# zahraamselim/compressed-rag-suite

Measured on AMD Instinct MI355X. Metric: queries/sec over N-vector corpus (exact cosine top-k; Recall@10 vs the exact fp32 ranking), higher is better.
Workload: dtype f16 x f16 -> f32; 1 GPU; c4; corpus_rows=10000000, rows_per_gpu=10000000, dim=384, queries_per_batch=64, distinct_queries_in_flight=2048, lanes=1 encoder + 1 search (encoder kernels <= 48 KB of LDS); 4 batches per sweep, batches_per_encoder_forward=16, searches_per_graph=4, top_k=10, k_scan=24, slab=f16, refine_fp32=True, exact_escalation=True, encoder_in_step=True, engine=rag._engine.RetrievalEngine (the object ContextRetriever.retrieve_batch drives), encoder=all-MiniLM-L6-v2 shape, seeded random weights

## Files before the change

### compressed-rag-suite_amd/csrc/scan.h

```cpp
#pragma once
#include <hip/hip_runtime.h>
#include <stdint.h>

namespace crs {

struct ScanArgs {
  const _Float16* q;
  const void* slab;
  const float* scales;
  float* part_scores;
  int* part_rows;
  unsigned* tau_shared;
  unsigned long long* stamps;
  int n_rows;
  int n_tiles;
  int nq;
  int k;
  int sched;
  int boot;
  int kp;
  int nwg;
  int nqb;
  unsigned* ticket;
  int t_dyn;
  int dyn_mask;
  int nt;
};

struct ExactWs {
  float* thr;
  int* cnt;
  int* done;
  int64_t* lists;
};

int refine_launch(const _Float16* q16, int nq, int pdim, const _Float16* slab, int n_rows, const float* win_s,
                  const int64_t* win, int k, int tile_rows, int64_t id_base, float* out_s, int64_t* out_i, hipStream_t stream);

int refine_i8_launch(const _Float16* q16, int nq, int pdim, const void* slab, const float* scales, int n_rows, const float* win_s,
                     const int64_t* win, int k, int tile_rows, int64_t id_base, float* out_s, int64_t* out_i, hipStream_t stream);

int scan_tile_rows(int pdim);
int scan_i8_tile_rows();
int scan_wg_per_cu();
bool scan_share_tau();
int scan_launch_f16(const ScanArgs& a, int pdim, int nwg, hipStream_t stream);
int scan_launch_i8(const ScanArgs& a, int pdim, int slots, hipStream_t stream);
int scan_tb_wg_per_cu(int pdim, int nw);
bool scan_tb_has_8_waves(int pdim);
int scan_launch_tb(const ScanArgs& a, int pdim, int nw, int slots, hipStream_t stream);
int scan_ticket_zero(unsigned* ticket, hipStream_t stream);
int scan_tb_long_chain_slots(int pdim, int nw, int k);
int scan_i8_long_chain_slots(int pdim, int k);
int scan_wide_waves(int nq, int k, int pdim);
bool scan_wide_streamed(int k);
int scan_wide_wg_per_cu(int nw, int pdim);
int scan_wide_slots(int k);
int scan_wide_tile_rows(int nw, int pdim);
int scan_launch_wide(const ScanArgs& a, int pdim, int nw, hipStream_t stream);

int scan_w1_queries_per_wg(int nq, int k, int pdim);
int scan_launch_w1(const ScanArgs& a, int pdim, hipStream_t stream);

int merge_slices(int nlists, int k_in);
int merge_launch_i32(const float* scores, const int* rows, int nlists, int nq, int k_in, int k_out,
                     int64_t id_base, float* out_scores, int64_t* out_ids, float* inter_s, int64_t* inter_i, hipStream_t stream);
int merge_launch_i64(const float* scores, const int64_t* ids, int nlists, int nq, int k_in, int k_out,
                     float* out_scores, int64_t* out_ids, hipStream_t stream);

int merge_launch_wire(const void* wire, size_t block_bytes, size_t scores_off, int nlists, int nq, int k_in, int k_out,
                      float* out_scores, int64_t* out_ids, hipStream_t stream);

int merge_sorted_launch_i64(const float* scores, const int64_t* ids, int nlists, int nq, int k_in, int k_out, float* out_scores,
                            int64_t* out_ids, hipStream_t stream);
int merge_sorted_launch_wire(const void* wire, size_t block_bytes, size_t scores_off, int nlists, int nq, int k_in, int k_out,
                             float* out_scores, int64_t* out_ids, hipStream_t stream);

int mmr_order_launch(const float* vecs, int64_t n_rows, int dim, const int64_t* rows, const double* rel, const int* counts, int nq,
                     int m_max, double lam, int* order, hipStream_t stream);

int rerank_lexical_launch(const float* scores, const int64_t* rows, int nq, int m_max, const int64_t* doc_off, const int* doc_tok,
                          int64_t n_rows, int64_t n_doc_tok, const int64_t* q_off, const int* q_tok, int64_t n_q_tok, const int* q_norm,
                          int k, double threshold, int* order, int* out_count, double* sim, double* rr, int* reranked, hipStream_t stream);

int token_match_launch(const float* a, const int* len_a, int seq_a, const float* b, const int* len_b, int seq_b, int n_pairs, int hidden,
                       const float* w_a, const float* w_b, float* out, hipStream_t stream);

int refine_f32_launch(const float* q32, int nq, int dim, const float* shadow, int64_t n_rows, int64_t id_base,
                      const int64_t* cand, int k_in, int k_out, float* out_s, int64_t* out_i, hipStream_t stream);
int slab_append_launch(const float* emb, int64_t n, int dim, int pdim, int slab_type, void* slab,
                       float* scales, float* shadow, int64_t row0, float* row_err_max, hipStream_t stream);
int queries_to_f16_launch(const float* q, int nq, int dim, int pdim, _Float16* out, hipStream_t stream);
int score_rows_launch(const float* q32, int nq, int dim, const float* shadow, int64_t n_rows, int64_t id_base, int k, const int64_t* ids,
                      float* scores, hipStream_t stream);
int rescore_launch(const float* q32, int nq, int dim, const float* shadow, int64_t n_rows,
                   int64_t id_base, int k, float* scores, int64_t* ids, hipStream_t stream);

bool finish_fits(int nlists, int kp, int kc, int tile_rows, int pdim);
int finish_cert_launch(const float* part_s, const int* part_r, int nlists, int kp, const _Float16* q16, int nq, int pdim,
                       const _Float16* slab, int n_rows, int tile_rows, const float* q32, int dim, const float* shadow, int64_t id_base,
                       int kc, int k_out, float err_rows, float* cand_s, int64_t* cand_i, float* out_s, int64_t* out_i, int* status,
                       const ExactWs& ws, hipStream_t stream);

float exact_err_arith(int dim, int pdim);
float exact_err_rows_bound(int dim, int slab_type);
int refine_cert_launch(const float* q32, const _Float16* q16, int nq, int dim, int pdim, int slab_type, const float* shadow,
                       int64_t n_rows, int64_t id_base, const int64_t* cand, const float* cand_s, int k_in, int k_out,
                       float err_rows, float* out_s, int64_t* out_i, int* status, const ExactWs& ws, hipStream_t stream);
int escalate_launch(const float* q32, const _Float16* q16, int nq, int dim, int pdim, int slab_type, const void* slab,
                    const float* scales, const float* shadow, int64_t n_rows, int64_t id_base, int k_out, float* out_s,
                    int64_t* out_i, int* status, const ExactWs& ws, int cap, int cus, hipStream_t stream);

int large_k_max_parts();
int large_cert_launch(const float* q32, const _Float16* q16, int nq, int dim, int pdim, int slab_type, const float* shadow, int64_t n_rows,
                      int64_t id_base, const int64_t* cand, const float* cand_s, int parts, int64_t chunk_rows, int k_out, float err_rows,
                      float* out_s, int64_t* out_i, int* status, const ExactWs& ws, hipStream_t stream);

}
```

### compressed-rag-suite_amd/csrc/scan_common.h

```cpp
#pragma once
#include <hip/hip_runtime.h>
#include <stdint.h>

#include "scan.h"
#include "lds_dma.h"

#define CRS_NSTREAMS (a.nwg)
#define CRS_QBLOCK (crs::grid_qblock(a))
#define CRS_STREAM (crs::grid_stream(a))

namespace crs {
namespace {

typedef _Float16 f16x8 __attribute__((ext_vector_type(8)));
typedef float f32x4 __attribute__((ext_vector_type(4)));
typedef unsigned u32x4 __attribute__((ext_vector_type(4)));

__device__ __forceinline__ int grid_qblock(const ScanArgs& a) {
  const int b = (int)blockIdx.x;
  if (a.nqb == 1) return 0;
  if (a.nwg & 7) return b % a.nqb;
  return (b >> 3) % a.nqb;
}
__device__ __forceinline__ int grid_stream(const ScanArgs& a) {
  const int b = (int)blockIdx.x;
  if (a.nqb == 1) return b;
  if (a.nwg & 7) return b / a.nqb;
  return ((b >> 3) / a.nqb) * 8 + (b & 7);
}


#ifdef CRS_STAMPS
#define CRS_STAMP(slot)                                                                          \
  do {                                                                                           \
    if (a.stamps && (threadIdx.x & 63) == 0) {                                                   \
      const unsigned long long t_ = __builtin_amdgcn_s_memtime();                               \
      a.stamps[((size_t)CRS_STREAM * 4 + (threadIdx.x >> 6)) * 64 + (slot)] = t_;                \
    }                                                                                            \
  } while (0)
#define CRS_STAMP_REAL(slot)                                                                     \
  do {                                                                                           \
    if (a.stamps && (threadIdx.x & 63) == 0)                                                     \
      a.stamps[((size_t)CRS_STREAM * 4 + (threadIdx.x >> 6)) * 64 + (slot)] = __builtin_amdgcn_s_memrealtime(); \
  } while (0)
#else
#define CRS_STAMP(slot) do {} while (0)
#define CRS_STAMP_REAL(slot) do {} while (0)

#endif

#ifdef CRS_STAMPS
#define WP_DECL unsigned long long wp_[12] = {0, 0, 0, 0, 0, 0, 0, 0, 0, 0, 0, 0}; unsigned long long wp_t_ = __builtin_amdgcn_s_memtime(); const unsigned long long wp_t0_ = wp_t_
#define WP_LAP(slot) do { const unsigned long long n_ = __builtin_amdgcn_s_memtime(); wp_[slot] += n_ - wp_t_; wp_t_ = n_; } while (0)
#define WP_COUNT(slot) do { ++wp_[slot]; } while (0)
#define WP_STORE(nw_) do { if (a.stamps && lane == 0) { wp_[11] = __builtin_amdgcn_s_memtime() - wp_t0_; for (int i_ = 0; i_ < 12; ++i_) a.stamps[((size_t)blockIdx.x * (nw_) + wave) * 12 + i_] = wp_[i_]; } } while (0)
#else
#define WP_DECL do {} while (0)
#define WP_LAP(slot) do {} while (0)
#define WP_COUNT(slot) do {} while (0)
#define WP_STORE(nw_) do {} while (0)
#endif

constexpr int kThreads = 256;
constexpr int kWaves = 4;
constexpr float kNegInf = -__builtin_huge_valf();

template <int L>
__device__ __forceinline__ void bitonic_sort_desc(float (&v)[L]) {
#pragma unroll
  for (int k = 2; k <= L; k <<= 1) {
#pragma unroll
    for (int j = k >> 1; j > 0; j >>= 1) {
#pragma unroll
      for (int i = 0; i < L; ++i) {
        const int l = i ^ j;
        if (l > i) {
          const bool desc = ((i & k) == 0);
          const float a = v[i], b = v[l];
          const float hi = fmaxf(a, b), lo = fminf(a, b);
          v[i] = desc ? hi : lo;
          v[l] = desc ? lo : hi;
        }
      }
    }
  }
}

template <int L>
__device__ __forceinline__ void bitonic_clean_desc(float (&v)[L]) {
#pragma unroll
  for (int j = L >> 1; j > 0; j >>= 1) {
#pragma unroll
    for (int i = 0; i < L; ++i) {
      const int l = i ^ j;
      if (l > i) {
        const float a = v[i], b = v[l];
        v[i] = fmaxf(a, b);
        v[l] = fminf(a, b);
      }
    }
  }
}

__device__ __forceinline__ int quad_sum(int x) {
  x += __shfl_xor(x, 16);
  x += __shfl_xor(x, 32);
  return x;
}
__device__ __forceinline__ int quad_min(int x) {
  x = min(x, __shfl_xor(x, 16));
  x = min(x, __shfl_xor(x, 32));
  return x;
}

template <int L>
__device__ __forceinline__ float pick(const float (&m)[L], int idx) {
  float t = m[0];
#pragma unroll
  for (int j = 1; j < L; ++j) t = fminf(t, (j <= idx) ? m[j] : __builtin_huge_valf());
  return t;
}

__device__ __forceinline__ float kth_of_quad(float (&s)[16], int k) {
  bitonic_sort_desc<16>(s);
  float m[16];
#pragma unroll
  for (int j = 0; j < 16; ++j) m[j] = fmaxf(s[j], __shfl_xor(s[15 - j], 16));
  bitonic_clean_desc<16>(m);
#pragma unroll
  for (int j = 0; j < 16; ++j) s[j] = fmaxf(m[j], __shfl_xor(m[15 - j], 32));
  bitonic_clean_desc<16>(s);
  return pick<16>(s, k - 1);
}

__device__ __forceinline__ float kth_of_quad(float (&s)[32], int k) {
  const int lane = threadIdx.x & 63;
  const bool upper = (lane >> 4) & 1;
  bitonic_sort_desc<32>(s);
  float m[32];
#pragma unroll
  for (int j = 0; j < 32; ++j) {
    const float o = __shfl_xor(s[31 - j], 16);
    m[j] = upper ? fminf(s[j], o) : fmaxf(s[j], o);
  }
  bitonic_clean_desc<32>(m);
#pragma unroll
  for (int j = 0; j < 32; ++j) s[j] = fmaxf(m[j], __shfl_xor(m[31 - j], 48));
#pragma unroll
  for (int j = 0; j < 32; ++j) {
    const float o = __shfl_xor(s[j], 16);
    m[j] = upper ? fminf(s[j], o) : fmaxf(s[j], o);
  }
  bitonic_clean_desc<32>(m);
  const float t = pick<32>(m, (k - 1) & 31);
  const int src = (lane & 47 & ~16) | (((k - 1) >> 5) << 4);
  return __shfl(t, src);
}

__device__ __forceinline__ float pair_max(float x) {
  const auto r = __builtin_amdgcn_permlane32_swap(__float_as_uint(x), __float_as_uint(x), false, false);
  return fmaxf(__uint_as_float(r[0]), __uint_as_float(r[1]));
}
__device__ __forceinline__ float quad_max(float x) {
  const auto r = __builtin_amdgcn_permlane16_swap(__float_as_uint(x), __float_as_uint(x), false, false);
  return pair_max(fmaxf(__uint_as_float(r[0]), __uint_as_float(r[1])));
}

__device__ __forceinline__ unsigned ord_of(float x) {
  const unsigned u = __float_as_uint(x);
  return (u & 0x80000000u) ? ~u : (u | 0x80000000u);
}
__device__ __forceinline__ float float_of_ord(unsigned o) {
  return __uint_as_float((o & 0x80000000u) ? (o & 0x7fffffffu) : ~o);
}
__device__ __forceinline__ float foreign_tau(unsigned o) {
  return o > 1u ? float_of_ord(o - 1u) : kNegInf;
}

template <int L, bool FINAL>
__device__ __forceinline__ void compact(float* __restrict__ sbuf, int* __restrict__ ibuf, int lane,
                                        int& cnt, float& tau, int k, float* out_s, int* out_i,
                                        bool q_valid, int kp = 0, unsigned* tau_pub = nullptr) {
  float v[L], s[L];
  int id[L];
#pragma unroll
  for (int j = 0; j < L; ++j) {
    const bool in = j < cnt;
    const float x = sbuf[j * 64 + lane];
    v[j] = in ? x : kNegInf;
    s[j] = v[j];
    id[j] = ibuf[j * 64 + lane];
  }
  const int total = quad_sum(cnt);
  float tnew = kth_of_quad(s, k);
  int n_gt = 0, n_eq = 0;
#pragma unroll
  for (int j = 0; j < L; ++j) {
    n_gt += (j < cnt && v[j] > tnew) ? 1 : 0;
    n_eq += (j < cnt && v[j] == tnew) ? 1 : 0;
  }
  n_gt = quad_sum(n_gt);
  n_eq = quad_sum(n_eq);
  int need = (total >= k) ? (k - n_gt) : n_eq;
  int idthr = 0x7fffffff;
  if (__any(n_eq > need)) {
    int thr = -1;
    const int rounds = (n_eq > need) ? need : 0;
    for (int it = 0; __any(it < rounds); ++it) {
      int c = 0x7fffffff;
#pragma unroll
      for (int j = 0; j < L; ++j)
        if (j < cnt && v[j] == tnew && id[j] > thr) c = min(c, id[j]);
      c = quad_min(c);
      if (it < rounds) thr = c;
    }
    if (n_eq > need) idthr = thr;
  }
  unsigned km = 0;
#pragma unroll
  for (int j = 0; j < L; ++j) {
    const bool keep = (j < cnt) && (v[j] > tnew || (v[j] == tnew && id[j] <= idthr));
    km |= (keep ? 1u : 0u) << j;
  }
  const int c = __popc(km);
  const int qb = lane & 15;
  const int c0 = __shfl(c, qb), c1 = __shfl(c, qb + 16), c2 = __shfl(c, qb + 32),
            c3 = __shfl(c, qb + 48);
  const int g = lane >> 4;
  const int prefix = (g > 0 ? c0 : 0) + (g > 1 ? c1 : 0) + (g > 2 ? c2 : 0);
  const int kept = c0 + c1 + c2 + c3;
  if (FINAL) {
    if (q_valid) {
#pragma unroll
      for (int j = 0; j < L; ++j) {
        if ((km >> j) & 1u) {
          const int p = prefix + __popc(km & ((1u << j) - 1u));
          out_s[p] = v[j];
          out_i[p] = id[j];
        }
      }
      for (int p = kept + g; p < kp; p += 4) {
        out_s[p] = kNegInf;
        out_i[p] = -1;
      }
    }
  } else {
#pragma unroll
    for (int j = 0; j < L; ++j) {
      if ((km >> j) & 1u) {
        const int p = prefix + __popc(km & ((1u << j) - 1u));
        const int dl = qb + ((p & 3) << 4);
        sbuf[(p >> 2) * 64 + dl] = v[j];
        ibuf[(p >> 2) * 64 + dl] = id[j];
      }
    }
    cnt = (kept - g + 3) >> 2;
    if (total >= k) {
      tau = fmaxf(tau, tnew);
      if (tau_pub && g == 0 && q_valid)
        __hip_atomic_fetch_max(tau_pub, ord_of(tnew), __ATOMIC_RELAXED, __HIP_MEMORY_SCOPE_AGENT);
    }
  }
}

template <int L>
__device__ __forceinline__ void flush_lists(float* __restrict__ sbuf, int* __restrict__ ibuf, int lane, int& cnt,
                                            float& tau, int k, int kp, float* out_s, int* out_i, bool q_valid) {
  const int total = quad_sum(cnt);
  if (__any(total > kp)) {
    compact<L, true>(sbuf, ibuf, lane, cnt, tau, k, out_s, out_i, q_valid, kp);
    return;
  }
  const int qb = lane & 15, g = lane >> 4;
  const int c0 = __shfl(cnt, qb), c1 = __shfl(cnt, qb + 16), c2 = __shfl(cnt, qb + 32);
  const int prefix = (g > 0 ? c0 : 0) + (g > 1 ? c1 : 0) + (g > 2 ? c2 : 0);
  if (!q_valid) return;
#pragma unroll
  for (int j = 0; j < L; ++j) {
    if (j < cnt) {
      out_s[prefix + j] = sbuf[j * 64 + lane];
      out_i[prefix + j] = ibuf[j * 64 + lane];
    }
  }
  for (int p = total + g; p < kp; p += 4) {
    out_s[p] = kNegInf;
    out_i[p] = -1;
  }
}

}
}
```

### compressed-rag-suite_amd/csrc/scan_wide.hip

```cpp

#include "scan_common.h"

#include <stdlib.h>

namespace crs {
int scan_wide_slots(int k);
namespace {

typedef float f32x16 __attribute__((ext_vector_type(16)));
typedef __attribute__((address_space(3))) void* lds_ptr_t;




template <int D, int NW>
constexpr int wide_rb() { return (NW == 8 && D <= 384) ? 2 : 1; }

template <int K>
constexpr bool wide_streamed() { return K > 16; }
template <int D, int NW, int K>
constexpr bool wide_stagger() { return NW == 8 && D <= 384 && !(D == 384 && K >= 16) && !(D == 256 && K >= 32); }

template <int D, int NW>
struct WCfg {
  static constexpr int kThreadsW = NW * 64;
  static constexpr int kCpr = D / 8;
  static constexpr int RB = wide_rb<D, NW>();
  static constexpr int TR = 32 * RB;
  static constexpr int kTileBytes = TR * D * 2;
  static constexpr int kLoads = kTileBytes / (kThreadsW * 16);
  static constexpr int kKsteps = D / 16;
  static constexpr int kQStage = NW * 4096;
  static constexpr int kLds = 2 * kTileBytes > kTileBytes + kQStage ? 2 * kTileBytes : kTileBytes + kQStage;
  static_assert(D % 128 == 0, "row length must be a multiple of 128 elements");
  static_assert(kTileBytes % (kThreadsW * 16) == 0, "tile must split into whole 16-byte loads");
};

template <int D, int NW, int K>
__global__ __launch_bounds__(NW * 64, 2) void scan_wide_kernel(const ScanArgs a) {
  using C = WCfg<D, NW>;
  constexpr int kT = C::kThreadsW;
  extern __shared__ __attribute__((aligned(16))) char smem[];
  char* tile_buf = smem;
  const int tid = threadIdx.x;
  const int lane = tid & 63;
  const int wave = __builtin_amdgcn_readfirstlane(tid >> 6);
  const int nwg = CRS_NSTREAMS;
  const int qblock = CRS_QBLOCK, stream = CRS_STREAM;
  WP_DECL;
  const bool wave_active = (qblock * (NW * 32) + wave * 32) < a.nq;

  unsigned src_off[C::kLoads];
#pragma unroll
  for (int j = 0; j < C::kLoads; ++j) {
    const int P = j * kT + tid;
    const int r = P / C::kCpr, cp = P % C::kCpr;
    src_off[j] = (unsigned)(r * C::kCpr + ((cp & ~15) | ((cp ^ r) & 15))) * 16u;
  }
  const char* slab = reinterpret_cast<const char*>(a.slab);
  const size_t last_chunk = (size_t)a.n_rows * (D * 2) - 16;
  constexpr int RB = C::RB, WTR = C::TR;
  const int n_full = a.n_rows / WTR;
  const unsigned lds_wave = __builtin_amdgcn_readfirstlane((unsigned)(size_t)(lds_ptr_t)tile_buf + (unsigned)wave * 1024u);
  auto dma_tile = [&](int tile_, int buf) {
    const int tile = __builtin_amdgcn_readfirstlane(tile_);
    const unsigned dst0 = lds_wave + (unsigned)(buf * C::kTileBytes);
    if (tile < n_full) {
      const char* base = uniform_ptr(slab + (size_t)tile * C::kTileBytes);
      if (wide_streamed<K>() && a.nt) {
#pragma unroll
        for (int j = 0; j < C::kLoads; ++j) lds_dma16_nt(dst0 + (unsigned)(j * kT * 16), src_off[j], base);
      } else {
#pragma unroll
        for (int j = 0; j < C::kLoads; ++j) lds_dma16(dst0 + (unsigned)(j * kT * 16), src_off[j], base);
      }
    } else {
#pragma unroll
      for (int j = 0; j < C::kLoads; ++j) {
        size_t off = (size_t)tile * C::kTileBytes + src_off[j];
        off = off > last_chunk ? last_chunk : off;
        const char* p = slab + off;
        const unsigned dst = dst0 + (unsigned)(j * kT * 16);
        lds_dma16(dst, p);
      }
    }
  };

  __shared__ int sh_next[2];
  constexpr bool kDyn = wide_streamed<K>();
  const int tend = a.n_tiles;
  const int t_dyn = kDyn ? a.t_dyn : a.n_tiles;
  int t = stream, t_prev = stream;
  int tn = t + nwg;
  dma_tile(t, 0);

  const int qn = lane & 31, h = lane >> 5;
  const int qi = qblock * (NW * 32) + wave * 32 + qn;
  const bool q_valid = qi < a.nq;
  f16x8 qf[C::kKsteps];
  {
    constexpr int kBlocks = C::kCpr / 8;
    constexpr int kGroup = 3;
    char* qs = tile_buf + C::kTileBytes + wave * 4096;
    const int q0 = qblock * (NW * 32) + wave * 32;
    const char* qbytes = reinterpret_cast<const char*>(a.q);
    const f16x8 z = {0, 0, 0, 0, 0, 0, 0, 0};
#pragma unroll
    for (int g0 = 0; g0 < kBlocks; g0 += kGroup) {
      u32x4 tmp[kGroup * 4];
#pragma unroll
      for (int p = 0; p < kGroup; ++p) {
        if (g0 + p < kBlocks) {
#pragma unroll
          for (int j = 0; j < 4; ++j) {
            const int c = j * 64 + lane, q = c >> 3, col = c & 7;
            const int qq = q0 + q < a.nq ? q0 + q : a.nq - 1;
            tmp[p * 4 + j] = *reinterpret_cast<const u32x4*>(qbytes + (size_t)qq * (D * 2) + (g0 + p) * 128 + col * 16);
          }
        }
      }
#pragma unroll
      for (int p = 0; p < kGroup; ++p) {
        if (g0 + p < kBlocks) {
#pragma unroll
          for (int j = 0; j < 4; ++j) {
            const int c = j * 64 + lane, q = c >> 3, col = c & 7;
            *reinterpret_cast<u32x4*>(qs + q * 128 + ((col ^ ((q >> 1) & 7)) * 16)) = tmp[p * 4 + j];
          }
#pragma unroll
          for (int ksl = 0; ksl < 4; ++ksl) {
            const int col = 2 * ksl + h;
            const f16x8 v = *reinterpret_cast<const f16x8*>(qs + qn * 128 + ((col ^ ((qn >> 1) & 7)) * 16));
            qf[(g0 + p) * 4 + ksl] = q_valid ? v : z;
          }
        }
      }
    }
#pragma unroll
    for (int ks = 0; ks < C::kKsteps; ++ks) {
      f16x8 x = qf[ks];
      asm volatile("" : "+v"(x));
      qf[ks] = x;
    }
  }
  int a_off[8];
#pragma unroll
  for (int j = 0; j < 8; ++j) a_off[j] = qn * (C::kCpr * 16) + (((2 * j + h) ^ qn) & 15) * 16;

  float ts[K];
  int tr[K];
#pragma unroll
  for (int j = 0; j < K; ++j) { ts[j] = kNegInf; tr[j] = -1; }

  float px = kNegInf;
  int pr = -1;
  auto insert = [&](float x, int xr) {
#pragma unroll
    for (int j = 0; j < K; ++j) {
      const bool c = x > ts[j];
      const float s_old = ts[j];
      const int r_old = tr[j];
      ts[j] = c ? x : s_old;
      tr[j] = c ? xr : r_old;
      x = c ? s_old : x;
      xr = c ? r_old : xr;
    }
  };

  asm volatile("s_waitcnt vmcnt(0)" ::: "memory");
  __syncthreads();
  WP_LAP(0);

  const bool late = wide_stagger<D, NW, K>() && wave >= 4;
  struct Acc { f32x16 a[RB]; };
  Acc acc_prev;
#pragma unroll
  for (int rb = 0; rb < RB; ++rb)
#pragma unroll
    for (int r = 0; r < 16; ++r) acc_prev.a[rb][r] = 0.f;
  auto sweep = [&](const char* buf) {
    Acc acc;
#pragma unroll
    for (int rb = 0; rb < RB; ++rb) {
#pragma unroll
      for (int r = 0; r < 16; ++r) acc.a[rb][r] = 0.f;
#pragma unroll
      for (int ks = 0; ks < C::kKsteps; ++ks) {
        const f16x8 af = *reinterpret_cast<const f16x8*>(buf + rb * 32 * (C::kCpr * 16) + a_off[ks & 7] + (ks >> 3) * 256);
        acc.a[rb] = __builtin_amdgcn_mfma_f32_32x32x16_f16(af, qf[ks], acc.a[rb], 0, 0, 0);
      }
    }
    return acc;
  };
  auto select = [&](const Acc& accs, int te, int ie) {
    float x = kNegInf;
#pragma unroll
    for (int rb = 0; rb < RB; ++rb) {
      const f32x16& acc = accs.a[rb];
      if (te < n_full) {
        const float m0 = __builtin_fmaxf(__builtin_fmaxf(acc[0], acc[1]), acc[2]);
        const float m1 = __builtin_fmaxf(__builtin_fmaxf(acc[3], acc[4]), acc[5]);
        const float m2 = __builtin_fmaxf(__builtin_fmaxf(acc[6], acc[7]), acc[8]);
        const float m3 = __builtin_fmaxf(__builtin_fmaxf(acc[9], acc[10]), acc[11]);
        const float m4 = __builtin_fmaxf(__builtin_fmaxf(acc[12], acc[13]), acc[14]);
        x = __builtin_fmaxf(x, __builtin_fmaxf(__builtin_fmaxf(__builtin_fmaxf(m0, m1), __builtin_fmaxf(m2, m3)), __builtin_fmaxf(m4, acc[15])));
      } else {
        const int row_base = te * WTR + rb * 32 + 4 * h;
#pragma unroll
        for (int r = 0; r < 16; ++r) {
          const int row = row_base + 8 * (r >> 2) + (r & 3);
          x = (row < a.n_rows) ? __builtin_fmaxf(x, acc[r]) : x;
        }
      }
    }
    x = pair_max(x);
    if ((ie & 1) == h) { px = x; pr = te * WTR; }
    if (ie & 1) {
      insert(px, pr);
      px = kNegInf;
      pr = -1;
    }
  };

  int cur = 0, it = 0;
  while (t < tend) {
    const bool has_next = tn < tend;
    if (has_next) dma_tile(tn, cur ^ 1);
    const bool in_dyn = kDyn && tn >= t_dyn;
    const bool draw = kDyn && a.ticket != nullptr && has_next && (in_dyn ? ((tn - t_dyn) & a.dyn_mask) == a.dyn_mask : tn + nwg >= t_dyn);
    unsigned tk = 0;
    if constexpr (kDyn) {
      const unsigned mask = __builtin_amdgcn_readfirstlane((draw && wave == 0) ? 1u : 0u);
      unsigned long long keep;
      const unsigned zero = 0u, one = 1u;
      asm volatile("s_mov_b64 %1, exec\n\ts_mov_b32 exec_lo, %2\n\ts_mov_b32 exec_hi, 0\n\tglobal_atomic_add %0, %3, %4, %5 sc0\n\ts_mov_b64 exec, %1"
                   : "+v"(tk), "=&s"(keep) : "s"(mask), "v"(zero), "v"(one), "s"(a.ticket) : "memory");
    }
    if (wave_active) {
      WP_LAP(1);
      const char* buf = tile_buf + cur * C::kTileBytes;
      if (!late) {
        const Acc acc = sweep(buf);
        WP_LAP(3);
        select(acc, t, it);
      } else {
        if (it > 0) select(acc_prev, t_prev, it - 1);
        WP_LAP(2);
        acc_prev = sweep(buf);
        WP_LAP(3);
      }
    }
    WP_LAP(4);
    int tnn = in_dyn ? tn + 1 : tn + nwg;
    if constexpr (kDyn) {
      asm volatile("s_waitcnt vmcnt(0)" : "+v"(tk) : : "memory");
      if (draw && tid == 0) sh_next[it & 1] = t_dyn + (int)tk * (a.dyn_mask + 1);
    } else {
      asm volatile("s_waitcnt vmcnt(0)" ::: "memory");
    }
    WP_LAP(6);
    __syncthreads();
    WP_LAP(7);
    if (kDyn && draw) {
      tnn = __builtin_amdgcn_readfirstlane(sh_next[it & 1]);
      tnn = (unsigned)tnn < (unsigned)tend ? tnn : tend;
    }
    cur ^= 1;
    ++it;
    t_prev = t;
    t = tn;
    tn = tnn;
  }

  if (wave_active && late && it > 0) select(acc_prev, t_prev, it - 1);
  if (wave_active && (it & 1)) insert(px, pr);
  if (wave_active && q_valid) {
    const size_t o = ((size_t)qi * nwg + stream) * a.kp + (size_t)h * K;
#pragma unroll
    for (int j = 0; j < K; ++j) {
      a.part_scores[o + j] = ts[j];
      a.part_rows[o + j] = tr[j];
    }
  }
  WP_LAP(10);
  WP_STORE(NW);
}

template <int D, int NW, int K>
int launch_wide(const ScanArgs& a, hipStream_t stream) {
  using C = WCfg<D, NW>;
  static bool done = false;
  auto kernel = &scan_wide_kernel<D, NW, K>;
  if (!done) {
    hipError_t e = hipFuncSetAttribute(reinterpret_cast<const void*>(kernel),
                                       hipFuncAttributeMaxDynamicSharedMemorySize, C::kLds);
    if (e != hipSuccess) return (int)e;
    done = true;
  }
  hipLaunchKernelGGL(kernel, dim3(a.nqb * a.nwg), dim3(NW * 64), C::kLds, stream, a);
  return (int)hipGetLastError();
}

template <int D, int NW>
int launch_wide_k(const ScanArgs& a, hipStream_t stream) {
  const int kk = scan_wide_slots(a.k);
  if (kk == 4) return launch_wide<D, NW, 4>(a, stream);
  if (kk == 10) return launch_wide<D, NW, 10>(a, stream);
  if (kk == 16) return launch_wide<D, NW, 16>(a, stream);
  if constexpr (D <= 384) {
    if (kk == 24) return launch_wide<D, NW, 24>(a, stream);
    if (kk == 32) return launch_wide<D, NW, 32>(a, stream);
  }
  return -1;
}

template <int D>
int launch_wide_d(const ScanArgs& a, int nw, hipStream_t stream) {
  return nw == 8 ? launch_wide_k<D, 8>(a, stream) : launch_wide_k<D, 4>(a, stream);
}

}

int scan_wide_waves(int nq, int k, int pdim) {
  static int on = -1;
  if (on < 0) {
    const char* e = getenv("CRS_SCAN_WIDE");
    on = (e && e[0] == '0') ? 0 : 1;
  }
  if (!on || nq <= 64 || k > 32 || pdim > 512 || (k > 16 && pdim > 384)) return 0;
  return nq > 128 ? 8 : 4;
}
int scan_wide_tile_rows(int nw, int pdim) { return (nw == 8 && pdim <= 384) ? 64 : 32; }
int scan_wide_slots(int k) { return k <= 4 ? 4 : k <= 10 ? 10 : k <= 16 ? 16 : k <= 24 ? 24 : 32; }
bool scan_wide_streamed(int k) { return scan_wide_slots(k) > 16; }
int scan_wide_wg_per_cu(int nw, int pdim) { return nw == 8 ? 1 : 2; }

int scan_launch_wide(const ScanArgs& a, int pdim, int nw, hipStream_t stream) {
  switch (pdim) {
    case 128: return launch_wide_d<128>(a, nw, stream);
    case 256: return launch_wide_d<256>(a, nw, stream);
    case 384: return launch_wide_d<384>(a, nw, stream);
    case 512: return launch_wide_d<512>(a, nw, stream);
    default: return -1;
  }
}

}
```

Before: 111,700 queries/s.

## Split wide-scan top-k slots across lane halves and enable stagger for K=24

For K>16 the wide scan kernel now keeps only K/2 top-k slots per lane. The two 32-lane halves form one combined list, and each new candidate is inserted with a shift that pulls the partner half's tail element across via permlane32_swap. This replaces the old pairing of alternate tiles and cuts per-lane register pressure and the insertion chain length. The unused second-half output slots are filled with -inf sentinels. It also turns on the late-wave stagger for D=384, NW=8, K=24, with an env toggle to disable it. The risk is that the split list may not hold the exact per-pair top-K, which could change the candidates passed to merging.

```diff
diff --git a/compressed-rag-suite_amd/csrc/scan.h b/compressed-rag-suite_amd/csrc/scan.h
--- a/compressed-rag-suite_amd/csrc/scan.h
+++ b/compressed-rag-suite_amd/csrc/scan.h
@@ -25,6 +25,7 @@
   int t_dyn;
   int dyn_mask;
   int nt;
+  int no_stagger;
 };
 
 struct ExactWs {
diff --git a/compressed-rag-suite_amd/csrc/scan_common.h b/compressed-rag-suite_amd/csrc/scan_common.h
--- a/compressed-rag-suite_amd/csrc/scan_common.h
+++ b/compressed-rag-suite_amd/csrc/scan_common.h
@@ -50,10 +50,10 @@
 #endif
 
 #ifdef CRS_STAMPS
-#define WP_DECL unsigned long long wp_[12] = {0, 0, 0, 0, 0, 0, 0, 0, 0, 0, 0, 0}; unsigned long long wp_t_ = __builtin_amdgcn_s_memtime(); const unsigned long long wp_t0_ = wp_t_
-#define WP_LAP(slot) do { const unsigned long long n_ = __builtin_amdgcn_s_memtime(); wp_[slot] += n_ - wp_t_; wp_t_ = n_; } while (0)
+#define WP_DECL unsigned wp_[12] = {0, 0, 0, 0, 0, 0, 0, 0, 0, 0, 0, 0}; unsigned wp_t_ = (unsigned)__builtin_amdgcn_s_memtime(); const unsigned wp_t0_ = wp_t_
+#define WP_LAP(slot) do { const unsigned n_ = (unsigned)__builtin_amdgcn_s_memtime(); wp_[slot] += n_ - wp_t_; wp_t_ = n_; } while (0)
 #define WP_COUNT(slot) do { ++wp_[slot]; } while (0)
-#define WP_STORE(nw_) do { if (a.stamps && lane == 0) { wp_[11] = __builtin_amdgcn_s_memtime() - wp_t0_; for (int i_ = 0; i_ < 12; ++i_) a.stamps[((size_t)blockIdx.x * (nw_) + wave) * 12 + i_] = wp_[i_]; } } while (0)
+#define WP_STORE(nw_) do { if (a.stamps && lane == 0) { wp_[11] = (unsigned)__builtin_amdgcn_s_memtime() - wp_t0_; for (int i_ = 0; i_ < 12; ++i_) a.stamps[((size_t)blockIdx.x * (nw_) + wave) * 12 + i_] = wp_[i_]; } } while (0)
 #else
 #define WP_DECL do {} while (0)
 #define WP_LAP(slot) do {} while (0)
diff --git a/compressed-rag-suite_amd/csrc/scan_wide.hip b/compressed-rag-suite_amd/csrc/scan_wide.hip
--- a/compressed-rag-suite_amd/csrc/scan_wide.hip
+++ b/compressed-rag-suite_amd/csrc/scan_wide.hip
@@ -18,8 +18,15 @@
 
 template <int K>
 constexpr bool wide_streamed() { return K > 16; }
+template <int K>
+constexpr bool wide_split() { return K > 16; }
+template <int K>
+constexpr int wide_lane_slots() { return wide_split<K>() ? K / 2 : K; }
 template <int D, int NW, int K>
-constexpr bool wide_stagger() { return NW == 8 && D <= 384 && !(D == 384 && K >= 16) && !(D == 256 && K >= 32); }
+constexpr bool wide_stagger() {
+  if (D == 384 && NW == 8 && K == 24) return true;
+  return NW == 8 && D <= 384 && !(D == 384 && K >= 16) && !(D == 256 && K >= 32);
+}
 
 template <int D, int NW>
 struct WCfg {
@@ -147,16 +154,18 @@
 #pragma unroll
   for (int j = 0; j < 8; ++j) a_off[j] = qn * (C::kCpr * 16) + (((2 * j + h) ^ qn) & 15) * 16;
 
-  float ts[K];
-  int tr[K];
-#pragma unroll
-  for (int j = 0; j < K; ++j) { ts[j] = kNegInf; tr[j] = -1; }
+  constexpr bool kSplit = wide_split<K>();
+  constexpr int KL = wide_lane_slots<K>();
+  float ts[KL];
+  int tr[KL];
+#pragma unroll
+  for (int j = 0; j < KL; ++j) { ts[j] = kNegInf; tr[j] = -1; }
 
   float px = kNegInf;
   int pr = -1;
   auto insert = [&](float x, int xr) {
 #pragma unroll
-    for (int j = 0; j < K; ++j) {
+    for (int j = 0; j < KL; ++j) {
       const bool c = x > ts[j];
       const float s_old = ts[j];
       const int r_old = tr[j];
@@ -167,11 +176,24 @@
     }
   };
 
+  auto insert_shift = [&](float x, float v, int vr) {
+#pragma unroll
+    for (int j = 0; j < KL; ++j) {
+      const bool c = x > ts[j];
+      const float s_old = ts[j];
+      const int r_old = tr[j];
+      ts[j] = c ? v : s_old;
+      tr[j] = c ? vr : r_old;
+      v = c ? s_old : v;
+      vr = c ? r_old : vr;
+    }
+  };
+
   asm volatile("s_waitcnt vmcnt(0)" ::: "memory");
   __syncthreads();
   WP_LAP(0);
 
-  const bool late = wide_stagger<D, NW, K>() && wave >= 4;
+  const bool late = wide_stagger<D, NW, K>() && wave >= 4 && !(kSplit && a.no_stagger);
   struct Acc { f32x16 a[RB]; };
   Acc acc_prev;
 #pragma unroll
@@ -214,11 +236,18 @@
       }
     }
     x = pair_max(x);
-    if ((ie & 1) == h) { px = x; pr = te * WTR; }
-    if (ie & 1) {
-      insert(px, pr);
-      px = kNegInf;
-      pr = -1;
+    if constexpr (kSplit) {
+      const float ps = __uint_as_float(__builtin_amdgcn_permlane32_swap(__float_as_uint(ts[KL - 1]), __float_as_uint(ts[KL - 1]), false, false)[0]);
+      const int prow = (int)__builtin_amdgcn_permlane32_swap((unsigned)tr[KL - 1], (unsigned)tr[KL - 1], false, false)[0];
+      const bool c = h && x > ps;
+      insert_shift(x, c ? ps : x, c ? prow : te * WTR);
+    } else {
+      if ((ie & 1) == h) { px = x; pr = te * WTR; }
+      if (ie & 1) {
+        insert(px, pr);
+        px = kNegInf;
+        pr = -1;
+      }
     }
   };
 
@@ -273,13 +302,26 @@
   }
 
   if (wave_active && late && it > 0) select(acc_prev, t_prev, it - 1);
-  if (wave_active && (it & 1)) insert(px, pr);
-  if (wave_active && q_valid) {
-    const size_t o = ((size_t)qi * nwg + stream) * a.kp + (size_t)h * K;
-#pragma unroll
-    for (int j = 0; j < K; ++j) {
-      a.part_scores[o + j] = ts[j];
-      a.part_rows[o + j] = tr[j];
+  if constexpr (kSplit) {
+    if (wave_active && q_valid) {
+      const size_t o = ((size_t)qi * nwg + stream) * a.kp + (size_t)h * KL;
+#pragma unroll
+      for (int j = 0; j < KL; ++j) {
+        a.part_scores[o + j] = ts[j];
+        a.part_rows[o + j] = tr[j];
+        a.part_scores[o + K + j] = kNegInf;
+        a.part_rows[o + K + j] = -1;
+      }
+    }
+  } else {
+    if (wave_active && (it & 1)) insert(px, pr);
+    if (wave_active && q_valid) {
+      const size_t o = ((size_t)qi * nwg + stream) * a.kp + (size_t)h * K;
+#pragma unroll
+      for (int j = 0; j < K; ++j) {
+        a.part_scores[o + j] = ts[j];
+        a.part_rows[o + j] = tr[j];
+      }
     }
   }
   WP_LAP(10);
@@ -335,7 +377,10 @@
 bool scan_wide_streamed(int k) { return scan_wide_slots(k) > 16; }
 int scan_wide_wg_per_cu(int nw, int pdim) { return nw == 8 ? 1 : 2; }
 
-int scan_launch_wide(const ScanArgs& a, int pdim, int nw, hipStream_t stream) {
+int scan_launch_wide(const ScanArgs& a_, int pdim, int nw, hipStream_t stream) {
+  ScanArgs a = a_;
+  const char* se = getenv("CRS_WIDE_STAGGER");
+  a.no_stagger = (se && se[0] == '0') ? 1 : 0;
   switch (pdim) {
     case 128: return launch_wide_d<128>(a, nw, stream);
     case 256: return launch_wide_d<256>(a, nw, stream);
```

Result: faster. 113,800 queries/s (median of 6 runs) (+1.9%).
